# trflorian/s3od

Measured on AMD Instinct MI355X. Metric: train images/sec (dinob 1024px bf16) at 1/2/4/8 GPU; infer masks/sec 1GPU, higher is better.
Workload: dtype bf16; 1 GPU; synth_sod train model=dinob 1024px bs=16/GPU fwd+focal_iou loss+bwd+AdamW; model=dinob (DINOv3 ViT-B/16 + DPT + 3-mask head), global_batch=16, image_size=1024, parallelism=dp1, rccl_world_size=1

## Files before the change

s3od_amd/csrc/gemm_q.hip:

```cpp
#include "gemm.hpp"

DEV int kc64_x(int r) { const int h = (r >> 2) & 3; return h ^ ((h & 1) << 1); }
typedef __attribute__((address_space(3))) const char lds_cchar;
DEV unsigned lds_addr(const char* p) { return (unsigned)(unsigned long)(lds_cchar*)p; }
DEV const char* lds_ptr(unsigned a) { return (const char*)(lds_cchar*)(unsigned long)a; }
typedef int i32x4_t __attribute__((ext_vector_type(4)));
DEV i32x4_t q_rsrc(const void* p, unsigned long bytes) {
  const unsigned long a = (unsigned long)p;
  return i32x4_t{(int)(unsigned)a, (int)((a >> 32) & 0xffff), (int)(unsigned)(bytes < BUF_MAX ? bytes : BUF_MAX), 0x00020000};
}
DEV void blds16s(i32x4_t r, unsigned voff, unsigned soff, unsigned lds_wave_base) {
  asm volatile("s_mov_b32 m0, %3\n\ts_nop 0\n\tbuffer_load_dwordx4 %0, %1, %2 offen lds"
               :: "v"(voff), "s"(r), "s"(soff), "s"(lds_wave_base) : "memory");
}
template <class L, bool KCL = L::KCL> struct KStep;
template <class L> struct KStep<L, true> {
  const bf16* pb; unsigned long nb; unsigned vo[4], vt[4]; int wb, klim, kpart;
  DEV void setup(const L& l, int t0, int tid, int klim_) {
    const int lane = tid & 63, wave = wave_id(), rem = l.nrows - t0;
    wb = wave * 4096;
    klim = klim_;
    kpart = (klim & 31) ? klim >> 5 : -1;
    pb = l.p + (long)t0 * l.ld;
    nb = rem > 0 ? ((unsigned long)(min(rem, 256) - 1) * l.ld + l.K) * 2 : 0;
    const int kel = ((lane & 3) ^ kc64_x(lane >> 2)) * 8;
#pragma unroll
    for (int i = 0; i < 4; i++) {
      const int r = (wave * 4 + i) * 16 + (lane >> 2);
      vo[i] = r < rem ? (unsigned)(((long)r * l.ld + kel) * 2) : BUF_OOB;
      vt[i] = (klim & ~31) + kel < klim ? vo[i] : BUF_OOB;
    }
  }
  DEV void piece(const L&, int ks, char* img, int i) const {
    const auto rs = q_rsrc(pb, ks * 32 < klim ? nb : 0);
    blds16s(rs, ks == kpart ? vt[i] : vo[i], (unsigned)ks * 64u, lds_addr(img) + wb + i * 1024);
  }
};
template <class L> struct KStep<L, false> {
  unsigned vo[4]; int wb; unsigned long tot;
  DEV void setup(const L& l, int t0, int tid, int klim) {
    const int lane = tid & 63, wave = wave_id();
    wb = wave * 4096;
    tot = klim > 0 ? ((unsigned long)(klim - 1) * l.ld + l.ncols) * 2 : 0;
#pragma unroll
    for (int i = 0; i < 4; i++) {
      const int k = wave * 8 + (lane >> 5) + 2 * i;
      const int cl = t0 + mc_logical_byte<512>(k, (lane & 31) * 16) / 2;
      vo[i] = cl < l.ncols ? (unsigned)(((long)k * l.ld + cl) * 2) : BUF_OOB;
    }
  }
  DEV void piece(const L& l, int ks, char* img, int i) const {
    const unsigned long e0 = (unsigned long)ks * 32 * l.ld * 2;
    const auto rs = q_rsrc((const char*)l.p + e0, e0 < tot ? tot - e0 : 0);
    blds16s(rs, vo[i], 0u, lds_addr(img) + wb + i * 1024);
  }
};
template <bool KCL> struct QFrag;
template <> struct QFrag<true> {
  unsigned a;
  DEV void init(const char* img, int lane, int half) {
    const int l = lane & 15;
    a = lds_addr(img) + half * 8192 + l * 64 + (((lane >> 4) ^ kc64_x(l)) << 4);
  }
  DEV void flip(int d) { a += d; }
  DEV bf16x8 read(int st01, int i) const { return *(const bf16x8*)(lds_ptr(a) + st01 * 32768 + i * 1024); }
};
template <> struct QFrag<false> {
  unsigned a[8];
  DEV void init(const char* img, int lane, int half) {
    const int g = lane >> 4, l = lane & 15, q = l >> 2, p = l & 3, gk = q | ((g & 1) << 2);
#pragma unroll
    for (int i = 0; i < 8; i++) a[i] = lds_addr(img) + (8 * g + q) * 512 + half * 256 + ((i ^ gk) << 5) + 8 * p;
  }
  DEV void flip(int d) {
#pragma unroll
    for (int i = 0; i < 8; i++) a[i] += d;
  }
  DEV bf16x8 read(int st01, int i) const {
    const char* s = lds_ptr(a[i]) + st01 * 32768;
    return read_tr_pair(s, s + 2048);
  }
};

namespace {
constexpr int Q_THREADS = 256, Q_BM = 256, Q_BN = 256, Q_IMG = 256 * 64, Q_STAGE = 2 * Q_IMG, Q_RING = 4, Q_LDT = Q_BN + 4;
constexpr int Q_LDS = (Q_RING * Q_STAGE > 128 * Q_LDT * 4) ? Q_RING * Q_STAGE : 128 * Q_LDT * 4;
static_assert(Q_LDS <= 160 * 1024, "q kernel LDS budget");
template <int V> using IC = std::integral_constant<int, V>;
template <class F, int... I> DEV void q_seq(F& f, std::integer_sequence<int, I...>) { (f(IC<I>{}), ...); }
template <int N, class F> DEV void q_for(F f) { q_seq(f, std::make_integer_sequence<int, N>{}); }
}

DEV void q_wait_lgkm0() { __builtin_amdgcn_s_waitcnt(0xC07F); }

template <class LA, class LB, class EPI>
__global__ void __launch_bounds__(Q_THREADS, 1) igemm_q_kernel(LA la, LB lb, EPI epi, int KTILES, int split, int group) {
  static_assert(LA::ROWS == 256 && LB::ROWS == 256 && LA::NIW == 8 && LB::NIW == 8, "q kernel: 256-row loaders on 4 waves");
  static_assert(!LA::RELU && !LB::RELU, "q kernel: no ReLU-on-load (a VALU write of a fragment inside the MFMA stream)");
  extern __shared__ __attribute__((aligned(16))) char smem[];
  const int tid = threadIdx.x, lane = tid & 63, wave = wave_id();
  const int wm = wave >> 1, wn = wave & 1;
  int m0, n0;
  {
    int mt, nt_;
    tile_of_block(group, mt, nt_);
    m0 = mt * Q_BM; n0 = nt_ * Q_BN;
  }
  const int per = (KTILES + split - 1) / split;
  const int kt0 = blockIdx.z * per, kt1 = min(KTILES, kt0 + per);
  const int ks0 = 2 * kt0, n = 2 * (kt1 - kt0);
  epi.prepare(blockIdx.z);
  const int klim = min(la.K, (ks0 + n) * 32);
  KStep<LA> sa; KStep<LB> sb;
  sa.setup(la, m0, tid, klim);
  sb.setup(lb, n0, tid, klim);
  QFrag<LA::KCL> qa; QFrag<LB::KCL> qb;
  qa.init(smem, lane, wm);
  qb.init(smem + Q_IMG, lane, wn);
  f32x4 acc[8][8];
#pragma unroll
  for (int i = 0; i < 8; i++)
#pragma unroll
    for (int j = 0; j < 8; j++) acc[i][j] = f32x4{0.f, 0.f, 0.f, 0.f};
  bf16x8 fa[2][8], fb[2][8];
  auto read_frag = [&](int buf, int st01, int f) {
    if (f < 8) fb[buf][f] = qb.read(st01, f);
    else fa[buf][f - 8] = qa.read(st01, f - 8);
  };
  auto dma_piece = [&](int ks, char* stage, int d) {
    if (d < 4) sa.piece(la, ks, stage, d);
    else sb.piece(lb, ks, stage + Q_IMG, d - 4);
  };
  constexpr int FPG = (LA::KCL || LB::KCL) ? 2 : 1;
  constexpr int D0 = 4 + 16 / FPG + 4, DS = 4;
  static_assert(D0 + 7 * DS < 64, "DMA pieces inside the block");
  auto kstep = [&](auto PC, int ks, char* stage, int flip) __attribute__((always_inline)) {
    constexpr int P = decltype(PC)::value;
    if constexpr (P == 1) { qa.flip(flip); qb.flip(flip); }
    q_wait_lgkm0();
    asm volatile("s_nop 1");
    q_for<64>([&](auto MC) __attribute__((always_inline)) {
      constexpr int m = decltype(MC)::value, i = m >> 3, j = m & 7;
      asm volatile("v_mfma_f32_16x16x32_bf16 %0, %1, %2, %0" : "+a"(acc[i][j]) : "v"(fb[P][j]), "v"(fa[P][i]));
      if constexpr (m == 3) { wait_vmcnt<16>(); raw_barrier(); }
      if constexpr (m >= 4 && m < 4 + 16 / FPG) {
#pragma unroll
        for (int u = 0; u < FPG; u++) read_frag(P ^ 1, P ^ 1, (m - 4) * FPG + u);
      }
      if constexpr (m >= D0 && (m - D0) % DS == 0 && (m - D0) / DS < 8) dma_piece(ks + 4, stage, (m - D0) / DS);
      __builtin_amdgcn_sched_barrier(0);
    });
    asm volatile("" :: "v"(fa[P][0]), "v"(fa[P][1]), "v"(fa[P][2]), "v"(fa[P][3]),
                 "v"(fa[P][4]), "v"(fa[P][5]), "v"(fa[P][6]), "v"(fa[P][7]), "v"(fb[P][0]), "v"(fb[P][1]),
                 "v"(fb[P][2]), "v"(fb[P][3]), "v"(fb[P][4]), "v"(fb[P][5]), "v"(fb[P][6]), "v"(fb[P][7]));
  };
  if (n > 0) {
#pragma unroll
    for (int q = 0; q < Q_RING; q++)
#pragma unroll
      for (int d = 0; d < 8; d++) dma_piece(ks0 + q, smem + q * Q_STAGE, d);
    wait_vmcnt<24>();
    raw_barrier();
#pragma unroll
    for (int f = 0; f < 16; f++) read_frag(0, 0, f);
    int pair = 0, flip = 2 * Q_STAGE;
    for (int s = 0; s < n; s += 2) {
      kstep(IC<0>{}, ks0 + s, smem + pair, flip);
      kstep(IC<1>{}, ks0 + s + 1, smem + pair + Q_STAGE, flip);
      pair ^= 2 * Q_STAGE; flip = -flip;
    }
  }
  asm volatile("s_nop 7\n\ts_nop 7\n\ts_nop 7" ::: "memory");
  vm_drain();
  float* ct = (float*)smem;
#pragma unroll
  for (int h = 0; h < 2; h++) {
    lds_barrier();
    if (wm == h) {
#pragma unroll
      for (int i = 0; i < 8; i++)
#pragma unroll
        for (int j = 0; j < 8; j++) {
          const int r = i * 16 + (lane & 15), c = wn * 128 + j * 16 + (lane >> 4) * 4;
          *(f32x4*)(ct + r * Q_LDT + c) = acc[i][j];
        }
    }
    lds_barrier();
    epi(ct, Q_LDT, m0 + h * 128, n0, tid, 128, Q_BN, Q_THREADS);
  }
}

template <class LA, class LB, class EPI>
int launch_igemm_q(LA la, LB lb, EPI epi, int M, int N, int KTILES, int split, int zdim_extra, hipStream_t st) {
  if (!la.buf_ok() || !lb.buf_ok()) {
    s3od_set_error("igemm_q: operand window too large for a buffer descriptor");
    return 22;
  }
  auto kfn = igemm_q_kernel<LA, LB, EPI>;
  static const bool attr = ((void)hipFuncSetAttribute((const void*)kfn, hipFuncAttributeMaxDynamicSharedMemorySize, Q_LDS), true);
  (void)attr;
  dim3 grid(cdiv(N, Q_BN), cdiv(M, Q_BM), split * zdim_extra);
  const int group = S3OD_KNOB("S3OD_GEMM_GROUP", 0);
  hipLaunchKernelGGL(kfn, grid, dim3(Q_THREADS), Q_LDS, st, la, lb, epi, KTILES, split, group);
  return s3od_check_launch("igemm_q");
}

typedef DenseKC<bf16, 256, 4> QKC;
typedef DenseMC<bf16, 256, 4> QMC;
template int launch_igemm_q<QKC, QKC, EpiStd<bf16, bf16, bf16>>(QKC, QKC, EpiStd<bf16, bf16, bf16>, int, int, int, int, int, hipStream_t);
template int launch_igemm_q<QKC, QKC, EpiStd<float, float, bf16>>(QKC, QKC, EpiStd<float, float, bf16>, int, int, int, int, int, hipStream_t);
template int launch_igemm_q<QKC, QKC, EpiStd<float, bf16, bf16>>(QKC, QKC, EpiStd<float, bf16, bf16>, int, int, int, int, int, hipStream_t);
template int launch_igemm_q<QKC, QKC, EpiStd<bf16, float, bf16>>(QKC, QKC, EpiStd<bf16, float, bf16>, int, int, int, int, int, hipStream_t);
template int launch_igemm_q<QKC, QMC, EpiStd<bf16, bf16, bf16>>(QKC, QMC, EpiStd<bf16, bf16, bf16>, int, int, int, int, int, hipStream_t);
template int launch_igemm_q<QKC, QMC, EpiStd<float, float, float>>(QKC, QMC, EpiStd<float, float, float>, int, int, int, int, int, hipStream_t);
template int launch_igemm_q<QMC, QMC, EpiWgradPart>(QMC, QMC, EpiWgradPart, int, int, int, int, int, hipStream_t);
template int launch_igemm_q<QMC, QMC, EpiWgrad>(QMC, QMC, EpiWgrad, int, int, int, int, int, hipStream_t);
```

Measured before the change: 110.4 images/s.

## Load K-contiguous operands as 128-byte lines per 64-wide k-tile in q GEMM

For K-contiguous operands, the GEMM now fetches a whole 64-wide k-tile at once as 128-byte row lines into a padded LDS layout with a new swizzle, instead of two 32-wide 64-byte images per k-step. The ring becomes a two-tile double buffer with a new schedule that spreads DMA pieces, waits and fragment reads across the two MFMA half-steps. Wider contiguous global loads and fewer descriptor issues should improve memory efficiency. In exchange the prefetch depth is shallower, and the hand-tuned issue schedule and partial-tile masking get more complex.

```diff
diff --git a/s3od_amd/csrc/gemm_q.hip b/s3od_amd/csrc/gemm_q.hip
--- a/s3od_amd/csrc/gemm_q.hip
+++ b/s3od_amd/csrc/gemm_q.hip
@@ -1,6 +1,12 @@
 #include "gemm.hpp"
 
-DEV int kc64_x(int r) { const int h = (r >> 2) & 3; return h ^ ((h & 1) << 1); }
+namespace {
+constexpr int Q_IMG = 256 * 64;
+constexpr int QL_BLK = 16 * 128 + 128, QL_HALF = 8 * 128 + 64;
+constexpr int QL_OPR = 16 * QL_BLK, QL_PAIR = 2 * QL_OPR;
+static_assert(QL_OPR >= 2 * Q_IMG, "an MC operand's two k-step images fit its region");
+}
+DEV int kcl_chunk(int l, int pc) { return (pc & 4) | ((pc & 3) ^ ((l >> 1) & 3)); }
 typedef __attribute__((address_space(3))) const char lds_cchar;
 DEV unsigned lds_addr(const char* p) { return (unsigned)(unsigned long)(lds_cchar*)p; }
 DEV const char* lds_ptr(unsigned a) { return (const char*)(lds_cchar*)(unsigned long)a; }
@@ -15,25 +21,25 @@
 }
 template <class L, bool KCL = L::KCL> struct KStep;
 template <class L> struct KStep<L, true> {
-  const bf16* pb; unsigned long nb; unsigned vo[4], vt[4]; int wb, klim, kpart;
+  const bf16* pb; unsigned long nb; unsigned vo[8], cut; int wb, klim, kcut;
   DEV void setup(const L& l, int t0, int tid, int klim_) {
     const int lane = tid & 63, wave = wave_id(), rem = l.nrows - t0;
-    wb = wave * 4096;
+    wb = wave * 4 * QL_BLK;
     klim = klim_;
-    kpart = (klim & 31) ? klim >> 5 : -1;
+    kcut = (klim & 63) ? klim >> 6 : -1;
     pb = l.p + (long)t0 * l.ld;
     nb = rem > 0 ? ((unsigned long)(min(rem, 256) - 1) * l.ld + l.K) * 2 : 0;
-    const int kel = ((lane & 3) ^ kc64_x(lane >> 2)) * 8;
-#pragma unroll
-    for (int i = 0; i < 4; i++) {
-      const int r = (wave * 4 + i) * 16 + (lane >> 2);
+    const int kel = kcl_chunk(lane >> 3, lane & 7) * 8;
+    cut = (klim & ~63) + kel < klim ? 0u : BUF_OOB;
+#pragma unroll
+    for (int i = 0; i < 8; i++) {
+      const int r = wave * 64 + i * 8 + (lane >> 3);
       vo[i] = r < rem ? (unsigned)(((long)r * l.ld + kel) * 2) : BUF_OOB;
-      vt[i] = (klim & ~31) + kel < klim ? vo[i] : BUF_OOB;
-    }
-  }
-  DEV void piece(const L&, int ks, char* img, int i) const {
-    const auto rs = q_rsrc(pb, ks * 32 < klim ? nb : 0);
-    blds16s(rs, ks == kpart ? vt[i] : vo[i], (unsigned)ks * 64u, lds_addr(img) + wb + i * 1024);
+    }
+  }
+  DEV void tile_piece(const L&, int kt, char* reg, int i) const {
+    const auto rs = q_rsrc(pb, kt * 64 < klim ? nb : 0);
+    blds16s(rs, vo[i] | (kt == kcut ? cut : 0u), (unsigned)kt * 128u, lds_addr(reg) + wb + (i >> 1) * QL_BLK + (i & 1) * QL_HALF);
   }
 };
 template <class L> struct KStep<L, false> {
@@ -54,18 +60,21 @@
     const auto rs = q_rsrc((const char*)l.p + e0, e0 < tot ? tot - e0 : 0);
     blds16s(rs, vo[i], 0u, lds_addr(img) + wb + i * 1024);
   }
+  DEV void tile_piece(const L& l, int kt, char* reg, int i) const { piece(l, 2 * kt + (i >> 2), reg + (i >> 2) * Q_IMG, i & 3); }
 };
 template <bool KCL> struct QFrag;
 template <> struct QFrag<true> {
+  static constexpr int KOFF = 64;
   unsigned a;
-  DEV void init(const char* img, int lane, int half) {
+  DEV void init(const char* reg, int lane, int half) {
     const int l = lane & 15;
-    a = lds_addr(img) + half * 8192 + l * 64 + (((lane >> 4) ^ kc64_x(l)) << 4);
+    a = lds_addr(reg) + half * 8 * QL_BLK + (l >> 3) * QL_HALF + (l & 7) * 128 + (kcl_chunk(l, lane >> 4) << 4);
   }
   DEV void flip(int d) { a += d; }
-  DEV bf16x8 read(int st01, int i) const { return *(const bf16x8*)(lds_ptr(a) + st01 * 32768 + i * 1024); }
+  DEV bf16x8 read(int off, int i) const { return *(const bf16x8*)(lds_ptr(a) + off + i * QL_BLK); }
 };
 template <> struct QFrag<false> {
+  static constexpr int KOFF = Q_IMG;
   unsigned a[8];
   DEV void init(const char* img, int lane, int half) {
     const int g = lane >> 4, l = lane & 15, q = l >> 2, p = l & 3, gk = q | ((g & 1) << 2);
@@ -76,19 +85,25 @@
 #pragma unroll
     for (int i = 0; i < 8; i++) a[i] += d;
   }
-  DEV bf16x8 read(int st01, int i) const {
-    const char* s = lds_ptr(a[i]) + st01 * 32768;
+  DEV bf16x8 read(int off, int i) const {
+    const char* s = lds_ptr(a[i]) + off;
     return read_tr_pair(s, s + 2048);
   }
 };
 
 namespace {
-constexpr int Q_THREADS = 256, Q_BM = 256, Q_BN = 256, Q_IMG = 256 * 64, Q_STAGE = 2 * Q_IMG, Q_RING = 4, Q_LDT = Q_BN + 4;
-constexpr int Q_LDS = (Q_RING * Q_STAGE > 128 * Q_LDT * 4) ? Q_RING * Q_STAGE : 128 * Q_LDT * 4;
-static_assert(Q_LDS <= 160 * 1024, "q kernel LDS budget");
+constexpr int Q_THREADS = 256, Q_BM = 256, Q_BN = 256, Q_STAGE = 2 * Q_IMG, Q_RING = 4, Q_LDT = Q_BN + 4;
+constexpr int q_max(int a, int b) { return a > b ? a : b; }
+template <bool LINES> constexpr int Q_LDS = q_max(LINES ? 2 * QL_PAIR : Q_RING * Q_STAGE, 128 * Q_LDT * 4);
+static_assert(Q_LDS<true> <= 160 * 1024 && Q_LDS<false> <= 160 * 1024, "q kernel LDS budget");
 template <int V> using IC = std::integral_constant<int, V>;
 template <class F, int... I> DEV void q_seq(F& f, std::integer_sequence<int, I...>) { (f(IC<I>{}), ...); }
 template <int N, class F> DEV void q_for(F f) { q_seq(f, std::make_integer_sequence<int, N>{}); }
+constexpr int QB_X = 8, QB_WAIT = 35, QB_RD[2] = {4, 36}, QB_DS = 4;
+constexpr int QB_D[2] = {QB_RD[0] + 8 + 2, QB_RD[1] + 8 + 2};
+constexpr int QB_NY = (63 - QB_D[1]) / QB_DS + 1, QB_NZ = 16 - QB_X - QB_NY;
+static_assert(4 + (QB_X - 1) * QB_DS < QB_WAIT && QB_WAIT < QB_RD[1], "pieces 0-7, then the wait, then the reads");
+static_assert(QB_NZ >= 0 && QB_D[0] + (QB_NZ - 1) * QB_DS < 64, "the last pieces of a tile inside the next block");
 }
 
 DEV void q_wait_lgkm0() { __builtin_amdgcn_s_waitcnt(0xC07F); }
@@ -97,6 +112,7 @@
 __global__ void __launch_bounds__(Q_THREADS, 1) igemm_q_kernel(LA la, LB lb, EPI epi, int KTILES, int split, int group) {
   static_assert(LA::ROWS == 256 && LB::ROWS == 256 && LA::NIW == 8 && LB::NIW == 8, "q kernel: 256-row loaders on 4 waves");
   static_assert(!LA::RELU && !LB::RELU, "q kernel: no ReLU-on-load (a VALU write of a fragment inside the MFMA stream)");
+  constexpr bool LINES = LA::KCL || LB::KCL;
   extern __shared__ __attribute__((aligned(16))) char smem[];
   const int tid = threadIdx.x, lane = tid & 63, wave = wave_id();
   const int wm = wave >> 1, wn = wave & 1;
@@ -114,60 +130,111 @@
   KStep<LA> sa; KStep<LB> sb;
   sa.setup(la, m0, tid, klim);
   sb.setup(lb, n0, tid, klim);
+  constexpr int B_OFF = LINES ? QL_OPR : Q_IMG;
   QFrag<LA::KCL> qa; QFrag<LB::KCL> qb;
   qa.init(smem, lane, wm);
-  qb.init(smem + Q_IMG, lane, wn);
+  qb.init(smem + B_OFF, lane, wn);
   f32x4 acc[8][8];
 #pragma unroll
   for (int i = 0; i < 8; i++)
 #pragma unroll
     for (int j = 0; j < 8; j++) acc[i][j] = f32x4{0.f, 0.f, 0.f, 0.f};
   bf16x8 fa[2][8], fb[2][8];
-  auto read_frag = [&](int buf, int st01, int f) {
-    if (f < 8) fb[buf][f] = qb.read(st01, f);
-    else fa[buf][f - 8] = qa.read(st01, f - 8);
+  auto read_frag = [&](int buf, int offa, int offb, int f) {
+    if (f < 8) fb[buf][f] = qb.read(offb, f);
+    else fa[buf][f - 8] = qa.read(offa, f - 8);
   };
-  auto dma_piece = [&](int ks, char* stage, int d) {
-    if (d < 4) sa.piece(la, ks, stage, d);
-    else sb.piece(lb, ks, stage + Q_IMG, d - 4);
+  auto mfma = [&](int P, int i, int j) __attribute__((always_inline)) {
+    asm volatile("v_mfma_f32_16x16x32_bf16 %0, %1, %2, %0" : "+a"(acc[i][j]) : "v"(fb[P][j]), "v"(fa[P][i]));
   };
-  constexpr int FPG = (LA::KCL || LB::KCL) ? 2 : 1;
-  constexpr int D0 = 4 + 16 / FPG + 4, DS = 4;
-  static_assert(D0 + 7 * DS < 64, "DMA pieces inside the block");
-  auto kstep = [&](auto PC, int ks, char* stage, int flip) __attribute__((always_inline)) {
-    constexpr int P = decltype(PC)::value;
-    if constexpr (P == 1) { qa.flip(flip); qb.flip(flip); }
-    q_wait_lgkm0();
-    asm volatile("s_nop 1");
-    q_for<64>([&](auto MC) __attribute__((always_inline)) {
-      constexpr int m = decltype(MC)::value, i = m >> 3, j = m & 7;
-      asm volatile("v_mfma_f32_16x16x32_bf16 %0, %1, %2, %0" : "+a"(acc[i][j]) : "v"(fb[P][j]), "v"(fa[P][i]));
-      if constexpr (m == 3) { wait_vmcnt<16>(); raw_barrier(); }
-      if constexpr (m >= 4 && m < 4 + 16 / FPG) {
-#pragma unroll
-        for (int u = 0; u < FPG; u++) read_frag(P ^ 1, P ^ 1, (m - 4) * FPG + u);
-      }
-      if constexpr (m >= D0 && (m - D0) % DS == 0 && (m - D0) / DS < 8) dma_piece(ks + 4, stage, (m - D0) / DS);
-      __builtin_amdgcn_sched_barrier(0);
-    });
+  auto keep_frags = [&](int P) __attribute__((always_inline)) {
     asm volatile("" :: "v"(fa[P][0]), "v"(fa[P][1]), "v"(fa[P][2]), "v"(fa[P][3]),
                  "v"(fa[P][4]), "v"(fa[P][5]), "v"(fa[P][6]), "v"(fa[P][7]), "v"(fb[P][0]), "v"(fb[P][1]),
                  "v"(fb[P][2]), "v"(fb[P][3]), "v"(fb[P][4]), "v"(fb[P][5]), "v"(fb[P][6]), "v"(fb[P][7]));
   };
-  if (n > 0) {
-#pragma unroll
-    for (int q = 0; q < Q_RING; q++)
-#pragma unroll
-      for (int d = 0; d < 8; d++) dma_piece(ks0 + q, smem + q * Q_STAGE, d);
-    wait_vmcnt<24>();
-    raw_barrier();
-#pragma unroll
-    for (int f = 0; f < 16; f++) read_frag(0, 0, f);
-    int pair = 0, flip = 2 * Q_STAGE;
-    for (int s = 0; s < n; s += 2) {
-      kstep(IC<0>{}, ks0 + s, smem + pair, flip);
-      kstep(IC<1>{}, ks0 + s + 1, smem + pair + Q_STAGE, flip);
-      pair ^= 2 * Q_STAGE; flip = -flip;
+  if constexpr (LINES) {
+    auto dma_piece = [&](int kt, char* pair, int d) {
+      if (d < 8) sa.tile_piece(la, kt, pair, d);
+      else sb.tile_piece(lb, kt, pair + QL_OPR, d - 8);
+    };
+    auto kstep = [&](auto PC, int kt, char* own, char* oth, int flip) __attribute__((always_inline)) {
+      constexpr int P = decltype(PC)::value;
+      if constexpr (P == 1) { qa.flip(flip); qb.flip(flip); }
+      q_wait_lgkm0();
+      asm volatile("s_nop 1");
+      q_for<64>([&](auto MC) __attribute__((always_inline)) {
+        constexpr int m = decltype(MC)::value, RD = QB_RD[P], D = QB_D[P];
+        mfma(P, m >> 3, m & 7);
+        if constexpr (P == 1 && m == 3) raw_barrier();
+        if constexpr (P == 1 && m >= 4 && (m - 4) % QB_DS == 0 && (m - 4) / QB_DS < QB_X) dma_piece(kt + 2, own, (m - 4) / QB_DS);
+        if constexpr (P == 1 && m == QB_WAIT) { wait_vmcnt<QB_X>(); raw_barrier(); }
+        if constexpr (m >= RD && m < RD + 8) {
+          constexpr int PN = P ^ 1;
+#pragma unroll
+          for (int u = 0; u < 2; u++)
+            read_frag(PN, PN * QFrag<LA::KCL>::KOFF, PN * QFrag<LB::KCL>::KOFF, (m - RD) * 2 + u);
+        }
+        if constexpr (m >= D && (m - D) % QB_DS == 0 && (m - D) / QB_DS < (P ? QB_NY : QB_NZ)) {
+          if constexpr (P == 1) dma_piece(kt + 2, own, QB_X + (m - D) / QB_DS);
+          else dma_piece(kt + 1, oth, QB_X + QB_NY + (m - D) / QB_DS);
+        }
+        __builtin_amdgcn_sched_barrier(0);
+      });
+      keep_frags(P);
+    };
+    if (n > 0) {
+#pragma unroll
+      for (int d = 0; d < 16; d++) dma_piece(kt0, smem, d);
+#pragma unroll
+      for (int d = 0; d < 16 - QB_NZ; d++) dma_piece(kt0 + 1, smem + QL_PAIR, d);
+      wait_vmcnt<16 - QB_NZ>();
+      raw_barrier();
+#pragma unroll
+      for (int f = 0; f < 16; f++) read_frag(0, 0, 0, f);
+      int pair = 0, flip = QL_PAIR;
+      for (int kt = kt0; kt < kt1; kt++) {
+        kstep(IC<0>{}, kt, smem + pair, smem + (QL_PAIR - pair), flip);
+        kstep(IC<1>{}, kt, smem + pair, smem + (QL_PAIR - pair), flip);
+        pair = QL_PAIR - pair; flip = -flip;
+      }
+    }
+  } else {
+    auto dma_piece = [&](int ks, char* stage, int d) {
+      if (d < 4) sa.piece(la, ks, stage, d);
+      else sb.piece(lb, ks, stage + Q_IMG, d - 4);
+    };
+    constexpr int D0 = 4 + 16 + 4, DS = 4;
+    static_assert(D0 + 7 * DS < 64, "DMA pieces inside the block");
+    auto kstep = [&](auto PC, int ks, char* stage, int flip) __attribute__((always_inline)) {
+      constexpr int P = decltype(PC)::value;
+      if constexpr (P == 1) { qa.flip(flip); qb.flip(flip); }
+      q_wait_lgkm0();
+      asm volatile("s_nop 1");
+      q_for<64>([&](auto MC) __attribute__((always_inline)) {
+        constexpr int m = decltype(MC)::value;
+        mfma(P, m >> 3, m & 7);
+        if constexpr (m == 3) { wait_vmcnt<16>(); raw_barrier(); }
+        if constexpr (m >= 4 && m < 4 + 16) read_frag(P ^ 1, (P ^ 1) * Q_STAGE, (P ^ 1) * Q_STAGE, m - 4);
+        if constexpr (m >= D0 && (m - D0) % DS == 0 && (m - D0) / DS < 8) dma_piece(ks + 4, stage, (m - D0) / DS);
+        __builtin_amdgcn_sched_barrier(0);
+      });
+      keep_frags(P);
+    };
+    if (n > 0) {
+#pragma unroll
+      for (int q = 0; q < Q_RING; q++)
+#pragma unroll
+        for (int d = 0; d < 8; d++) dma_piece(ks0 + q, smem + q * Q_STAGE, d);
+      wait_vmcnt<24>();
+      raw_barrier();
+#pragma unroll
+      for (int f = 0; f < 16; f++) read_frag(0, 0, 0, f);
+      int pair = 0, flip = 2 * Q_STAGE;
+      for (int s = 0; s < n; s += 2) {
+        kstep(IC<0>{}, ks0 + s, smem + pair, flip);
+        kstep(IC<1>{}, ks0 + s + 1, smem + pair + Q_STAGE, flip);
+        pair ^= 2 * Q_STAGE; flip = -flip;
+      }
     }
   }
   asm volatile("s_nop 7\n\ts_nop 7\n\ts_nop 7" ::: "memory");
@@ -197,11 +264,12 @@
     return 22;
   }
   auto kfn = igemm_q_kernel<LA, LB, EPI>;
-  static const bool attr = ((void)hipFuncSetAttribute((const void*)kfn, hipFuncAttributeMaxDynamicSharedMemorySize, Q_LDS), true);
+  constexpr int LDS = Q_LDS<LA::KCL || LB::KCL>;
+  static const bool attr = ((void)hipFuncSetAttribute((const void*)kfn, hipFuncAttributeMaxDynamicSharedMemorySize, LDS), true);
   (void)attr;
   dim3 grid(cdiv(N, Q_BN), cdiv(M, Q_BM), split * zdim_extra);
   const int group = S3OD_KNOB("S3OD_GEMM_GROUP", 0);
-  hipLaunchKernelGGL(kfn, grid, dim3(Q_THREADS), Q_LDS, st, la, lb, epi, KTILES, split, group);
+  hipLaunchKernelGGL(kfn, grid, dim3(Q_THREADS), LDS, st, la, lb, epi, KTILES, split, group);
   return s3od_check_launch("igemm_q");
 }
 
```

Result: no change. 110.4 images/s (median of 3 runs) (-0.0%).
